# erikszasz/GaussianSplattingRegistration

Hardware: AMD Instinct MI355X
Metric: Gaussians/sec through HEM level + ICP iters/sec, 2x5M-splat pair (higher is better)
Workload: dtype f32 (HEM) / f64 (ICP)

## Files before the change

gaussiansplattingregistration_amd/csrc/hem_select.h:

```cpp
#pragma once
#include "hem_device.h"

namespace gsr {

struct ParentRec;
struct SelectArgs {
    const float4* A;
    const float4* geo;
    const float* Rs;
    const unsigned* plist;
    const unsigned* porder;
    int xcd;
    const int* nheavy;
    int own_lo, own_hi;
    const int* cellStart;
    const float4* Ac;
    const int* cellStartC;
    const int* cellStartI;
    const double* logtab;
    const int* irank;
    const unsigned* ipos;
    int n_irr;
    int ell;
    const GridParams* gp;
// ... 84 lines not shown
    const float kf = 0.5f * (s2 - lf);
    const float margin = 1e-6f * (1.0f + fabsf(lf) + fabsf(s2));
    bool reject = kf > thr;
    const bool need_exact = !(qf >= 4.0f * FLT_MIN && qf <= 0.25f * FLT_MAX) || !(fabsf(s2) <= FLT_MAX) || !(fabsf(kf - thr) > margin);
    if (need_exact) {
        const float k = 0.5f * (s2 - glibc_logf_tab(det_c / det_p, logtab));
        reject = k > thr;
    }
    if (lf_out) *lf_out = lf;
    if (exact_out) *exact_out = need_exact;
    return reject;
}


template <bool IRR>
__device__ __forceinline__ void select_row_span(const SelectArgs& a, const GridParams& g, const f3& pm, const EllClip& ec, bool clip,
                                                float Ra2, int x0, int x1, int ry, int rz, int& s, int& len) {
    const bool edge = ry == 0 || ry == g.gy - 1 || rz == 0 || rz == g.gz - 1;
    const float ylo = ry == 0 ? -FLT_MAX : g.oy + ry * g.c - g.slack, yhi = ry == g.gy - 1 ? FLT_MAX : g.oy + (ry + 1) * g.c + g.slack;
    const float zlo = rz == 0 ? -FLT_MAX : g.oz + rz * g.c - g.slack, zhi = rz == g.gz - 1 ? FLT_MAX : g.oz + (rz + 1) * g.c + g.slack;
    const float dy = fmaxf(0.0f, fmaxf(ylo - pm.y, pm.y - yhi));
    const float dz = fmaxf(0.0f, fmaxf(zlo - pm.z, pm.z - zhi));
    const float rem = Ra2 - dy * dy - dz * dz;
    if (rem >= 0.0f) {
        const float hx = fast_sqrt(rem) * 1.00001f + g.slack;
        float lo = -hx, hi = hx;
        if (clip && !edge) {
            const float cy = 0.5f * (ylo + yhi) - pm.y, cz = 0.5f * (zlo + zhi) - pm.z;
            const float hy = 0.5f * (yhi - ylo), hz = 0.5f * (zhi - zlo);
            const float sc = fast_sqrt(fmaxf(0.0f, ec.k11 * cy * cy + 2.0f * ec.k12 * cy * cz + ec.k22 * cz * cz));
            const float smin = fmaxf(0.0f, sc * 0.999f - ec.kr * fast_sqrt(hy * hy + hz * hz));
// ... 3 lines not shown
            } else {
                const float w = fast_sqrt(rem2 * ec.im00) * 1.001f;
                const float t1 = ec.m01 * cy, t2 = ec.m02 * cz;
                const float xc = -(t1 + t2) * ec.im00;
                const float dl = (fabsf(ec.m01) * hy + fabsf(ec.m02) * hz) * ec.im00 * 1.001f;
                const float pad = g.slack + 1e-5f * fabsf(xc) + 1e-6f * (fabsf(t1) + fabsf(t2)) * ec.im00;
                lo = fmaxf(lo, xc - dl - w - pad);
                hi = fminf(hi, xc + dl + w + pad);
            }
        }
        if (lo <= hi) {
            int xa = cell_of(pm.x + lo, g.ox, g.inv_c, g.gx), xb = cell_of(pm.x + hi, g.ox, g.inv_c, g.gx);
            xa = xa < x0 ? x0 : xa;
            xb = xb > x1 ? x1 : xb;
            const int rowbase = (rz * g.gy + ry) * g.gx;
            int e;
            if (IRR) { s = a.cellStartI[rowbase + xa]; e = a.cellStartI[rowbase + xb + 1]; }
            else { s = a.cellStartC[rowbase + xa]; e = a.cellStartC[rowbase + xb + 1]; }
            len = e - s;
        }
    }
}

__device__ __forceinline__ void make_filter(const s6& Mf, float det_p, float kldThr, int ell, bool parent_regular, ParentRec& pr) {
    EllClip ec;
    ec.on = 0.0f; ec.k11 = ec.k12 = ec.k22 = ec.kr = ec.im00 = ec.m01 = ec.m02 = 0.0f; ec.T = __builtin_inff();
    pr.white = 0.0f;
    pr.u00 = pr.u01 = pr.u02 = pr.u11 = pr.u12 = pr.u22 = 0.0f;
    pr.T1 = __builtin_inff();
    pr.ey = pr.ez = __builtin_inff();
    const double thr2 = 2.0 * (double)kldThr;
    if (parent_regular && thr2 >= 0.0 && thr2 < 1e30) {
        const double m00 = Mf.e00, m01 = Mf.e01, m02 = Mf.e02, m11 = Mf.e11, m12 = Mf.e12, m22 = Mf.e22;
        double detM;
// ... 63 lines not shown
```

gaussiansplattingregistration_amd/csrc/hem_select.hip:

```cpp
#include "hem_select.h"

namespace gsr {

#ifdef GSR_SELECT_PROFILE
__device__ unsigned long long g_sel_prof[1024 * 16];
#endif
struct __attribute__((aligned(16))) ParLds {
    float4 r0;
    float4 r1;
    float4 r2;
    float4 r3;
    float R2;
    int js;
    int64_t base;
};
static_assert(sizeof(ParLds) == 80, "ParLds is read as four float4 and two 8-byte words");

#define SEL_Q3CAP 128
struct Q3 {
    unsigned *j, *rel;
    float *d2, *cd, *op, *det;
    int h, n;
};

__device__ __forceinline__ void select_stage3(const SelectArgs& a, const ParLds* par, int lane, int cnt, Q3& q3) {
    if (lane < cnt) {
        const int k = (q3.h + lane) & (SEL_Q3CAP - 1);
        const unsigned e = q3.j[k];
        const ParLds* pl = par + (e >> SEL_TAG_SHIFT);
        const float distanceDiff = sqrtf(q3.d2[k]);
        const float cdiff = sqrtf(q3.cd[k]);
        const float distWeight = expf(-distanceDiff * distanceDiff / a.tau2);
        const float colorInfluence = expf(-cdiff * cdiff / a.tau2);
        const float L = distWeight * q3.op[k] * colorInfluence * sqrtf(q3.det[k]);
        const int64_t dst = pl->base + (int64_t)q3.rel[k];
        a.pair_child[dst] = e & SEL_TAG_MASK;
        a.pair_wl[dst] = pl->r3.z * ref_clamp(L, FLT_MIN, 1e8f);
    }
    q3.h = (q3.h + cnt) & (SEL_Q3CAP - 1);
    q3.n -= cnt;
}

template <int MODE>
__device__ __forceinline__ void select_stage2(const SelectArgs& a, const ParLds* par, int lane, int cnt, const unsigned* q, int qh,
                                              unsigned& count_v, Q3& q3) {
    SEL_PROF_T(tp2);
    SEL_PROF_CNT(8, 1, lane); SEL_PROF_CNT(9, cnt, lane);
    bool acc = false;
    unsigned e = 0u;
    int k = 0;
    float d2 = 0.0f, cdiff = 0.0f, op = 0.0f, det_c = 0.0f;
    if (lane < cnt) {
        e = q[(qh + lane) & (SEL_QCAP - 1)];
        const int j = (int)(e & SEL_TAG_MASK);
        k = (int)(e >> SEL_TAG_SHIFT);
        const ParLds* pl = par + k;
        const float4 p0 = pl->r0, p1 = pl->r1;
        const float R2 = pl->R2;
        const float4* row = a.geo + 4 * (int64_t)j;
        float4 ca = row[0], cb = row[1], cc = row[2], cd = row[3];
        asm volatile("" : "+v"(ca.x), "+v"(ca.y), "+v"(ca.z), "+v"(ca.w), "+v"(cb.x), "+v"(cb.y), "+v"(cb.z), "+v"(cb.w),
                          "+v"(cc.x), "+v"(cc.y), "+v"(cc.z), "+v"(cc.w), "+v"(cd.x), "+v"(cd.y), "+v"(cd.z), "+v"(cd.w));
        const f3 cm = {ca.x, ca.y, ca.z};
        const f3 ccol = {cc.z, cc.w, cd.x};
        const f3 pm = {p0.x, p0.y, p0.z}, pcol = {p0.w, p1.x, p1.y};
        const f3 d = sub3(cm, pm);
        d2 = dot3(d, d);
        const f3 dc = sub3(ccol, pcol);
        cdiff = dot3(dc, dc);
        if (d2 < R2 && !(cdiff > a.colorThr2)) {
            const float4 p2 = pl->r2, p3 = pl->r3;
            const s6 ccov = {cb.x, cb.y, cb.z, cb.w, cc.x, cc.y};
            const s6 pinv = {p1.z, p1.w, p2.x, p2.y, p2.z, p2.w};
            det_c = cd.w;
            op = cd.y;
            const float smd = dot3(d, mul6(pinv, d));
            const float tr = trace_prod6(pinv, ccov);
            const float s2 = smd + tr - 3.0f;
            if (!kl_gate_rejects(s2, det_c, p3.x, p3.y, a.kldThr, a.logtab)) {
                const bool child_is_parent = (__float_as_uint(ca.w) & 1u) != 0u;
                acc = !(child_is_parent && j != pl->js);
            }
        }
    }
    const unsigned long long m = __ballot(acc);
    const int na = __popcll(m);
    SEL_PROF_CNT(15, na, lane);
    if (na == 0) { SEL_PROF_ADD(2, tp2, lane); return; }
    const int k_lo = __builtin_amdgcn_readfirstlane(k);
    const int k_hi = __builtin_amdgcn_readlane(k, __builtin_amdgcn_readfirstlane(cnt - 1));
    unsigned rel = 0u;
#pragma unroll
    for (int kk = 0; kk < SEL_NP; ++kk) {
        if (kk < k_lo || kk > k_hi) continue;
        const unsigned long long mk = __ballot(acc && k == kk);
        const unsigned ck = (unsigned)__builtin_amdgcn_readlane((int)count_v, kk);
        if (acc && k == kk) rel = ck + (unsigned)mbcnt64(mk, 0);
        if (lane == kk) count_v += (unsigned)__popcll(mk);
    }
    if (MODE == SEL_COUNT) { SEL_PROF_ADD(2, tp2, lane); return; }
    if (acc) {
        const int t = mbcnt64(m, q3.h + q3.n) & (SEL_Q3CAP - 1);
        q3.j[t] = e; q3.rel[t] = rel; q3.d2[t] = d2; q3.cd[t] = cdiff; q3.op[t] = op; q3.det[t] = det_c;
    }
    q3.n += na;
    __builtin_amdgcn_wave_barrier();
    if (q3.n >= 64) select_stage3(a, par, lane, 64, q3);
    __builtin_amdgcn_wave_barrier();
    SEL_PROF_ADD(2, tp2, lane);
}

__global__ __launch_bounds__(256) void k_parent_prep(int P, const unsigned* __restrict__ plist, const float4* __restrict__ geo,
                                                     const float* __restrict__ Rs, float kldThr, int ell, ParentRec* __restrict__ prec) {
    __shared__ ParentRec s_pr[4][64];
    const int lane = threadIdx.x & 63, wv = threadIdx.x >> 6;
    for (int base = blockIdx.x * blockDim.x + (threadIdx.x & ~63); base < P; base += gridDim.x * blockDim.x) {
        const int p = base + lane;
        if (p < P) {
        ParentRec pr;
        pr.js = (int)plist[p];
        const float4* prow = geo + 4 * (int64_t)pr.js;
        const float4 pa = prow[0], pb = prow[1], pc = prow[2], pd = prow[3];
// ... 11 lines not shown
        pr.active = (pr.R2 > 0.0f && pm_finite) ? 1 : 0;
        pr.selfq = (pr.active && (__float_as_uint(pa.w) & 2u)) ? 1 : 0;
        pr.rows = 0;
        s_pr[wv][lane] = pr;
        }
        __builtin_amdgcn_wave_barrier();
        const int nrec = P - base < 64 ? P - base : 64;
        const float4* src = reinterpret_cast<const float4*>(s_pr[wv]);
        float4* dst = reinterpret_cast<float4*>(prec + base);
        for (int t = lane; t < nrec * (int)(sizeof(ParentRec) / 16); t += 64) dst[t] = src[t];
        __builtin_amdgcn_wave_barrier();
    }
}

template <int MODE, bool IRR>
__device__ __forceinline__ void select_scan(const SelectArgs& a, const GridParams& g, const ParentRec& pr, const ParLds* par, unsigned ktag,
                                            const float (&vc)[11], int lane, unsigned long long* bits, unsigned* q, int& qh, int& qn, unsigned& count_v,
                                            Q3& q3, unsigned& cum, unsigned lo, unsigned hi, const int2* rl, int lcnt) {
    const f3 pm = pr.pm;
    const EllClip& ec = pr.ec;
    const bool listed = rl != nullptr;
    bool clip = false;
    int x0 = 0, x1 = 0, y0 = 0, z0 = 0, ny = 1, nrows = lcnt;
    float Ra2 = 0.0f;
    if (!listed) {
        int vz;
        asm volatile("v_mov_b32 %0, 0" : "=v"(vz));
        const auto uni = [vz](int v) { return __builtin_amdgcn_readfirstlane(v + vz); };
        const auto unif = [vz](float v) { return __builtin_bit_cast(float, __builtin_amdgcn_readfirstlane(__builtin_bit_cast(int, v) + vz)); };
        const float Ra = unif(fabsf(pr.R) * 1.00001f + g.slack);
        clip = !IRR && ec.on != 0.0f;
        const float Ry = clip ? fminf(Ra, pr.ey + g.slack) : Ra, Rz = clip ? fminf(Ra, pr.ez + g.slack) : Ra;
        x0 = uni(cell_of(pm.x - Ra, g.ox, g.inv_c, g.gx)); x1 = uni(cell_of(pm.x + Ra, g.ox, g.inv_c, g.gx));
        y0 = uni(cell_of(pm.y - Ry, g.oy, g.inv_c, g.gy));
        const int y1 = uni(cell_of(pm.y + Ry, g.oy, g.inv_c, g.gy));
        z0 = uni(cell_of(pm.z - Rz, g.oz, g.inv_c, g.gz));
        const int z1 = uni(cell_of(pm.z + Rz, g.oz, g.inv_c, g.gz));
        ny = y1 - y0 + 1;
        nrows = ny * (z1 - z0 + 1);
        Ra2 = unif(Ra * Ra);
    }
    const bool white = !IRR && pr.white != 0.0f;
    SEL_PROF_CNT(10, nrows, lane);
    for (int rb = 0; rb < nrows; rb += 64) {
        SEL_PROF_T(tpr);
        SEL_PROF_CNT(11, 1, lane);
        const int r = rb + lane;
        int s = 0, len = 0;
        if (r < nrows) {
            if (listed) { const int2 e = rl[r]; s = e.x; len = e.y; }
            else select_row_span<IRR>(a, g, pm, ec, clip, Ra2, x0, x1, y0 + r % ny, z0 + r / ny, s, len);
        }
        len = len > 0 ? len : 0;
        const unsigned long long nz_m = __ballot(len > 0);
        if (nz_m == 0ull) continue;
        const int incl = wave_incl_scan(len);
        const int pre = incl - len;
        const int total = __builtin_amdgcn_readlane(incl, 63);
        const unsigned cum0 = cum;
        cum += (unsigned)total;
        if (hi <= cum0 || lo >= cum) continue;
        const int b_lo = lo > cum0 ? (int)(lo - cum0) : 0;
        const int b_hi = hi - cum0 < (unsigned)total ? (int)(hi - cum0) : total;
        const int nrb = __popcll(nz_m);
        const int below = mbcnt64(nz_m, 0);
        const int dst = len > 0 ? below : nrb + (lane - below);
// ... 9 lines not shown
            const int seg_end = b_hi < seg0 + SEL_MCAP ? b_hi : seg0 + SEL_MCAP;
            for (int t0 = seg0; t0 < seg_end; t0 += 64 * SEL_U) {
                SEL_PROF_CNT(14, 1, lane);
                SEL_PROF_T(tps);
                float4 ca[SEL_U];
                int jj[SEL_U];
                int left[SEL_U];
#pragma unroll
                for (int u = 0; u < SEL_U; ++u) {
                    const int c0 = t0 + 64 * u;
                    const unsigned long long word = uniform64(bits[(c0 - seg0) >> 6]);
                    const int row = mbcnt64(word >> 1, rows_before - 1 + (int)(word & 1ull));
                    rows_before += __popcll(word);
                    left[u] = seg_end - c0;
                    const int k = c0 + lane + __builtin_amdgcn_ds_bpermute(row << 2, delta);
                    if (IRR) { jj[u] = lane < left[u] ? (int)a.ipos[k] : pr.js; ca[u] = a.A[jj[u]]; }
                    else { jj[u] = k; ca[u] = a.Ac[k]; }
                }
#pragma unroll
                for (int u = 0; u < SEL_U; ++u) {
                    if (left[u] <= 0) continue;
                    const f3 cm = {ca[u].x, ca[u].y, ca[u].z};
                    bool in;
                    if (white) {
                        in = !(white_smd(vc, cm.x, cm.y, cm.z) > vc[9]);
                    } else {
                        const f3 dq = sub3(pm, cm);
                        in = dot3(dq, dq) < pr.R2;
                    }
                    if (!IRR) {
                        in = in && (__float_as_uint(ca[u].w) & 2u);
                        jj[u] = (int)(__float_as_uint(ca[u].w) >> 2);
                    } else {
                        in = in && (!(__float_as_uint(ca[u].w) & 1u) || jj[u] == pr.js);
                    }
                    in = in && lane < left[u];
                    const unsigned long long m = __ballot(in);
                    if (m == 0ull) continue;
                    if (in) q[mbcnt64(m, qh + qn) & (SEL_QCAP - 1)] = (unsigned)jj[u] | ktag;
                    qn += __popcll(m);
                }
                __builtin_amdgcn_wave_barrier();
                SEL_PROF_ADD(4, tps, lane);
                while (qn >= 64) {
                    select_stage2<MODE>(a, par, lane, 64, q, qh, count_v, q3);
                    qh = (qh + 64) & (SEL_QCAP - 1);
                    qn -= 64;
                }
                __builtin_amdgcn_wave_barrier();
            }
            if (mine) bits[rel >> 6] = 0ull;
            __builtin_amdgcn_wave_barrier();
        }
    }
}

__device__ __forceinline__ void select_fill_par(const SelectArgs& a, int p, int64_t base, ParLds* slot) {
    const float4* r = reinterpret_cast<const float4*>(a.prec + p);
    const float4 r0 = r[0], r1 = r[1], r2 = r[2], r3 = r[3];
    slot->r0 = r0; slot->r1 = r1; slot->r2 = r2; slot->r3 = r3;
    slot->R2 = a.prec[p].R2; slot->js = a.prec[p].js; slot->base = base;
}

template <int MODE>
__device__ __forceinline__ void select_parent(const SelectArgs& a, const GridParams& g, int p, int k, unsigned lo, unsigned hi, int lane,
                                              const ParLds* par, unsigned* q, int& qh, int& qn, unsigned long long* bits, unsigned& count_v, Q3& q3) {
    SEL_PROF_T(tp0);
    ParentRec pr;
    {
        typedef unsigned u16v __attribute__((ext_vector_type(16)));
        typedef unsigned u8v __attribute__((ext_vector_type(8)));
        u16v w0, w1; u8v w2;
        const ParentRec* rp = a.prec + p;
        asm volatile("s_load_dwordx16 %0, %3, 0x0\n\ts_load_dwordx16 %1, %3, 0x40\n\ts_load_dwordx8 %2, %3, 0x80\n\ts_waitcnt lgkmcnt(0)"
                     : "=&s"(w0), "=&s"(w1), "=&s"(w2) : "s"(rp) : "memory");
        unsigned raw[40];
        static_assert(sizeof(raw) == sizeof(ParentRec), "the three scalar loads cover the record");
#pragma unroll
        for (int i = 0; i < 16; ++i) { raw[i] = w0[i]; raw[16 + i] = w1[i]; }
#pragma unroll
        for (int i = 0; i < 8; ++i) raw[32 + i] = w2[i];
        __builtin_memcpy(&pr, raw, sizeof(pr));
    }
    float vc[11];
    {
        const float src[11] = {pr.pm.x, pr.pm.y, pr.pm.z, pr.u00, pr.u01, pr.u02, pr.u11, pr.u12, pr.u22, pr.T1, 0.0f};
#pragma unroll
        for (int i = 0; i < 11; ++i) asm volatile("v_mov_b32 %0, %1" : "=v"(vc[i]) : "s"(src[i]));
    }
    const unsigned ktag = (unsigned)k << SEL_TAG_SHIFT;
    unsigned cum = 0;
    if (pr.selfq) {
        cum = 1u;
        if (lo == 0u) {
            if (lane == 0) q[(qh + qn) & (SEL_QCAP - 1)] = (unsigned)pr.js | ktag;
            qn += 1;
        }
        __builtin_amdgcn_wave_barrier();
        if (qn >= 64) {
            select_stage2<MODE>(a, par, lane, 64, q, qh, count_v, q3);
            qh = (qh + 64) & (SEL_QCAP - 1);
            qn -= 64;
        }
    }
    if (pr.active) {
        const int cA = pr.rows & 0xff, cB = (pr.rows >> 8) & 0xff;
        const int2* rlp = (a.rowlist != nullptr && pr.rows < 0) ? a.rowlist + (int64_t)p * (2 * SEL_ROWS) : nullptr;
        select_scan<MODE, false>(a, g, pr, par, ktag, vc, lane, bits, q, qh, qn, count_v, q3, cum, lo, hi,
                                 rlp != nullptr && cA <= SEL_ROWS ? rlp : nullptr, cA);
        if (a.n_irr > 0) select_scan<MODE, true>(a, g, pr, par, ktag, vc, lane, bits, q, qh, qn, count_v, q3, cum, lo, hi,
                                                 rlp != nullptr && cB <= SEL_ROWS ? rlp + SEL_ROWS : nullptr, cB);
    }
    SEL_PROF_ADD(0, tp0, lane);
    SEL_PROF_CNT(7, 1, lane);
}

template <int MODE>
__device__ __forceinline__ void select_flush(const SelectArgs& a, const ParLds* par, int lane, const unsigned* q, int& qh, int& qn,
                                             unsigned& count_v, Q3& q3) {
    while (qn > 0) {
        const int c = qn < 64 ? qn : 64;
        select_stage2<MODE>(a, par, lane, c, q, qh, count_v, q3);
        qh = (qh + c) & (SEL_QCAP - 1);
        qn -= c;
    }
    SEL_PROF_T(tp3);
    if ((MODE == SEL_FILL || MODE == SEL_SPARSE) && q3.n > 0) select_stage3(a, par, lane, q3.n, q3);
    SEL_PROF_ADD(3, tp3, lane);
    __builtin_amdgcn_wave_barrier();
}

template <int MODE, int WPB, bool QUEUE>
__global__ __launch_bounds__(64 * WPB) void k_select(SelectArgs a) {
    __shared__ unsigned s_q[WPB][SEL_QCAP];
    __shared__ unsigned s_q3u[WPB][2][SEL_Q3CAP];
    __shared__ float s_q3f[WPB][4][SEL_Q3CAP];
    __shared__ unsigned long long s_bits[WPB][SEL_MCAP / 64 + SEL_U];
    __shared__ ParLds s_par[WPB][SEL_NP];
    const int lane = threadIdx.x & 63, wv = __builtin_amdgcn_readfirstlane((int)(threadIdx.x >> 6));
    a.logtab = k_logf_tab;
    if (lane < SEL_MCAP / 64 + SEL_U) s_bits[wv][lane] = 0ull;
    unsigned* q = s_q[wv];
    ParLds* par = s_par[wv];
    Q3 q3 = {s_q3u[wv][0], s_q3u[wv][1], s_q3f[wv][0], s_q3f[wv][1], s_q3f[wv][2], s_q3f[wv][3], 0, 0};
    __builtin_amdgcn_wave_barrier();
    const GridParams g = *a.gp;
    int qh = 0, qn = 0;

    if constexpr (QUEUE) {
        const int n_items = a.hq[0];
        const unsigned part = *a.part_p;
        int item = (int)blockIdx.x * WPB + wv;
        while (item < n_items) {
            const uint2 it = a.hitem[item];
            const int p = __builtin_amdgcn_readfirstlane((int)a.porder[it.x]);
            const unsigned lo = (unsigned)__builtin_amdgcn_readfirstlane((int)(it.y * part));
            const unsigned hi = lo + part > lo ? lo + part : 0xffffffffu;
            int64_t base = 0;
            if (MODE == SEL_SPARSE) base = a.poff[p] + lo;
            if (MODE == SEL_SPARSE && a.cap_pairs && (unsigned long long)base + part > a.cap_pairs) {
                if (lane == 0) { a.part_cnt[item] = 0u; *a.abort_p = 1; }
                int nxt0 = 0;
                if (lane == 0) nxt0 = atomicAdd(&a.hq[1], 1);
                item = __builtin_amdgcn_readfirstlane(nxt0);
                continue;
            }
            if (MODE == SEL_FILL) {
                base = a.poff[p];
                for (int k = a.hfirst[p]; k < item; ++k) base += a.part_cnt[k];
            }
            unsigned count_v = 0u;
            if (lane == 0) select_fill_par(a, p, base, par);
            __builtin_amdgcn_wave_barrier();
            select_parent<MODE>(a, g, p, 0, lo, hi, lane, par, q, qh, qn, s_bits[wv], count_v, q3);
            select_flush<MODE>(a, par, lane, q, qh, qn, count_v, q3);
            if (lane == 0 && (MODE == SEL_COUNT || MODE == SEL_SPARSE)) {
                a.part_cnt[item] = count_v;
                atomicAdd(&a.pcnt[p], count_v);
            }
            int nxt = 0;
            if (lane == 0) nxt = atomicAdd(&a.hq[1], 1);
            item = __builtin_amdgcn_readfirstlane(nxt);
            __builtin_amdgcn_wave_barrier();
        }
    } else {
        SEL_PROF_T(tpk);
        const int np = a.np;
        const int ppb = WPB * np;
        const int nheavy = a.nheavy ? *a.nheavy : 0;
        const int nblk = (a.P + ppb - 1) / ppb;
        const int hb = ((nheavy + ppb - 1) / ppb + 7) & ~7;
        const int bid = block_slot((int)blockIdx.x, nblk, hb < nblk ? hb : nblk, a.xcd);
        if (bid < 0) return;
        const int slot0 = (bid * WPB + wv) * np;
        int p_v = -1;
        if (lane < np) {
// ... 9 lines not shown
                    } else {
                        p_v = p;
                        select_fill_par(a, p, base, par + lane);
                    }
                }
            }
        }
        unsigned long long todo = __ballot(p_v >= 0);
        unsigned count_v = 0u;
        __builtin_amdgcn_wave_barrier();
        SEL_PROF_ADD(5, tpk, lane);
        while (todo != 0ull) {
            const int k = __builtin_ctzll(todo);
            todo &= todo - 1ull;
            const int p = __builtin_amdgcn_readlane(p_v, k);
            select_parent<MODE>(a, g, p, k, 0u, 0xffffffffu, lane, par, q, qh, qn, s_bits[wv], count_v, q3);
        }
        SEL_PROF_T(tpf);
        select_flush<MODE>(a, par, lane, q, qh, qn, count_v, q3);
        SEL_PROF_ADD(6, tpf, lane);
        if (p_v >= 0 && (MODE == SEL_COUNT || MODE == SEL_SPARSE)) a.pcnt[p_v] = count_v;
    }
}

__global__ __launch_bounds__(256) void k_spans(SelectArgs a) {
    const int sub = threadIdx.x & 15;
    const int p = (int)(((int64_t)blockIdx.x * blockDim.x + threadIdx.x) >> 4);
    if (p >= a.P) return;
    unsigned long long scanned = 0;
    int selfq = 0;
    int nA = 0, nB = 0;
    if (p >= a.own_lo && p < a.own_hi) {
        const GridParams g = *a.gp;
        const float4* rq = reinterpret_cast<const float4*>(a.prec + p);
        float4 q0 = rq[0], q3 = rq[3], q6 = rq[6], q7 = rq[7], q8 = rq[8], q9 = rq[9];
        asm volatile("" : "+v"(q0.x), "+v"(q0.y), "+v"(q0.z), "+v"(q3.w), "+v"(q6.y), "+v"(q6.z), "+v"(q6.w), "+v"(q7.x), "+v"(q7.y), "+v"(q7.z), "+v"(q7.w),
// ... 14 lines not shown
            }
            n += __popc(gm);
        };
        if (rp->active) {
            const float Ra = fabsf(rp->R) * 1.00001f + g.slack;
            const float Ra2 = Ra * Ra;
            const int x0 = cell_of(pm.x - Ra, g.ox, g.inv_c, g.gx), x1 = cell_of(pm.x + Ra, g.ox, g.inv_c, g.gx);
            {
                const bool clip = ec.on != 0.0f;
                const float Ry = clip ? fminf(Ra, rp->ey + g.slack) : Ra, Rz = clip ? fminf(Ra, rp->ez + g.slack) : Ra;
                const int y0 = cell_of(pm.y - Ry, g.oy, g.inv_c, g.gy), y1 = cell_of(pm.y + Ry, g.oy, g.inv_c, g.gy);
                const int z0 = cell_of(pm.z - Rz, g.oz, g.inv_c, g.gz), z1 = cell_of(pm.z + Rz, g.oz, g.inv_c, g.gz);
                const int ny = y1 - y0 + 1, nrows = ny * (z1 - z0 + 1);
                for (int r = sub; r < nrows; r += 16) {
                    int s = 0, len = 0;
                    select_row_span<false>(a, g, pm, ec, clip, Ra2, x0, x1, y0 + r % ny, z0 + r / ny, s, len);
                    scanned += (unsigned long long)(len > 0 ? len : 0);
                    keep_span(0, s, len, nA);
                }
            }
            if (a.n_irr > 0) {
                const int y0 = cell_of(pm.y - Ra, g.oy, g.inv_c, g.gy), y1 = cell_of(pm.y + Ra, g.oy, g.inv_c, g.gy);
                const int z0 = cell_of(pm.z - Ra, g.oz, g.inv_c, g.gz), z1 = cell_of(pm.z + Ra, g.oz, g.inv_c, g.gz);
                const int ny = y1 - y0 + 1, nrows = ny * (z1 - z0 + 1);
                for (int r = sub; r < nrows; r += 16) {
                    int s = 0, len = 0;
                    select_row_span<true>(a, g, pm, ec, false, Ra2, x0, x1, y0 + r % ny, z0 + r / ny, s, len);
                    scanned += (unsigned long long)(len > 0 ? len : 0);
                    keep_span(1, s, len, nB);
                }
            }
        }
    }
    for (int o = 8; o > 0; o >>= 1) scanned += __shfl_xor(scanned, o);
    if (selfq) scanned += 1ull;
    if (sub == 0) {
        a.pcap[p] = (unsigned)(scanned > 0xffffffffull ? 0xffffffffull : scanned);
        if (a.rowlist) const_cast<ParentRec*>(a.prec)[p].rows = (int)(0x80000000u | (unsigned)(nA > SEL_ROWS ? 0xff : nA) | ((unsigned)(nB > SEL_ROWS ? 0xff : nB) << 8));
    }
}

void launch_parent_prep(hipStream_t st, int P, const unsigned* plist, const float4* geo, const float* Rs, float kldThr, int ell, ParentRec* prec) {
// ... 40 lines not shown
```

gaussiansplattingregistration_amd/csrc/icp.hip:

```cpp
#include "gsr_common.h"
#include "gsr_normals.h"
#include "gsr_solve.h"
#include "gsr_features.h"
#include "gsr_oneshot.h"

#include <float.h>
#include <math.h>
#include <stdlib.h>
#include <string.h>
#include <chrono>
#include <vector>

#include <rocprim/rocprim.hpp>

namespace gsr {
#ifndef GSR_ICP_MERGE_BS
#define GSR_ICP_MERGE_BS 1024
#define GSR_ICP_MERGE_IPT 4
#endif
using icp_merge_cfg = rocprim::merge_sort_config<512, GSR_ICP_MERGE_BS, GSR_ICP_MERGE_IPT, 128, 128, 4>;
using icp_sort_cfg = rocprim::radix_sort_config<rocprim::default_config, icp_merge_cfg,
                                                rocprim::radix_sort_onesweep_config<rocprim::kernel_config<1024, 16>, rocprim::kernel_config<1024, 16>, 11,
                                                                                    rocprim::block_radix_rank_algorithm::match>>;

// ... 194 lines not shown
    const double d = ((v < lo && k > 0) ? lo - v : ((v > hi && k < g - 1) ? v - hi : 0.0)) * 0.999999999 - eps;
    return d > 0.0 ? d : 0.0;
}

__device__ __forceinline__ void icp_consider(const float4 q, int j, double px, double py, double pz, double& bd, int& best, unsigned& best_i) {
    const double dx = px - (double)q.x, dy = py - (double)q.y, dz = pz - (double)q.z;
    const double d2 = dx * dx + dy * dy + dz * dz;
    const unsigned qi = __float_as_uint(q.w);
    if (d2 < bd || (d2 == bd && qi < best_i)) { bd = d2; best = j; best_i = qi; }
}

#define ICP_BLOCK_CROWDED 24
#ifndef ICP_ROW_BATCH
#define ICP_ROW_BATCH 4
#endif
template <int BLOCK>
__device__ __forceinline__ int icp_nearest(const IcpGrid& g, const int* __restrict__ cellStart,
                                           const float4* __restrict__ Tq, double px, double py, double pz, double& best_d2,
                                           double bound2 = 1.0 / 0.0) {
    int best = -1;
    unsigned best_i = 0xffffffffu;
    double bd = bound2;
    if (!(px == px) || !(py == py) || !(pz == pz)) { best_d2 = 1.0 / 0.0; return -1; }
    {
        const double ex = fmax(fmax(g.bx0 - px, px - g.bx1), 0.0), ey = fmax(fmax(g.by0 - py, py - g.by1), 0.0), ez = fmax(fmax(g.bz0 - pz, pz - g.bz1), 0.0);
        if ((ex * ex + ey * ey + ez * ez) * 0.999999999 >= bound2) { best_d2 = bound2; return -1; }
    }
    const int cx = icp_cell(px, g.ox, g.inv_c, g.gx), cy = icp_cell(py, g.oy, g.inv_c, g.gy), cz = icp_cell(pz, g.oz, g.inv_c, g.gz);
    const double eps = 1e-13 * (fabs(px) + fabs(py) + fabs(pz) + fabs(g.ox) + fabs(g.oy) + fabs(g.oz) + g.c * (double)(g.gx + g.gy + g.gz));
    int r0 = 0;
    if (BLOCK == 1 && g.rings >= 1) {
        int rs[9], re[9];
        const int xa = cx - 1 > 0 ? cx - 1 : 0, xb = cx + 1 < g.gx - 1 ? cx + 1 : g.gx - 1;
#pragma unroll
        for (int t = 0; t < 9; ++t) {
            const int z = cz + t / 3 - 1, y = cy + t % 3 - 1;
            const bool ok = z >= 0 && z < g.gz && y >= 0 && y < g.gy;
            const int rowbase = ok ? (z * g.gy + y) * g.gx : 0;
            rs[t] = ok ? cellStart[rowbase + xa] : 0;
            re[t] = ok ? cellStart[rowbase + xb + 1] : 0;
// ... 709 lines not shown


struct IcpState {
    double T[16];
    double fit, rmse;
    double ctr[3], nsg, rel_fit, rel_rmse;
    int iters, done, max_iter, kind, evals;
};

__device__ __forceinline__ bool icp_state_done(const IcpState* st) { return st->done != 0; }
__device__ __forceinline__ void icp_state_T(const IcpState* st, double T[12]) {
#pragma unroll
    for (int i = 0; i < 12; ++i) T[i] = st->T[i];
}

template <int KIND, int BLOCK, int FUSE>
__global__ __launch_bounds__(256, (FUSE != 0 && KIND != 2) ? 3 : 1) void k_icp_accumulate_dev(int64_t ns, const float* __restrict__ src, IcpState* st,
                                                            IcpGrid g, const int* __restrict__ cellStart, const int* __restrict__ nn_j,
                                                            const float4* __restrict__ Tq, const double* __restrict__ Tn,
                                                            const double* __restrict__ Sc, ColorArgs ca, double max_corr2,
                                                            int loss, double kparam, double* partials, unsigned* ticket,
                                                            double* acc_out, int nb_logical) {
    constexpr int fuse = FUSE;
    constexpr bool PERSIST = FUSE == 3;
    constexpr int NACC = KIND == 0 ? 17 : 30;
    __shared__ int s_last;
    __shared__ int s_stop;
    __shared__ double s_x[8][GSR_ICP_ACC_LEN];
    __shared__ IcpState s_st;
    const IcpRange rg = icp_block_range(ns, nb_logical < 0 ? -nb_logical : nb_logical, FUSE == 0 && nb_logical > 0);
    for (unsigned ev = 0;; ++ev) {
    double T[12];
    if constexpr (PERSIST) {
        if (threadIdx.x == 0) s_stop = __hip_atomic_load(&st->done, __ATOMIC_RELAXED, __HIP_MEMORY_SCOPE_AGENT) | (int)__hip_atomic_load(ticket + 2, __ATOMIC_RELAXED, __HIP_MEMORY_SCOPE_AGENT);
        __syncthreads();
        if (s_stop) return;
#pragma unroll
        for (int i = 0; i < 12; ++i) T[i] = __hip_atomic_load(&st->T[i], __ATOMIC_RELAXED, __HIP_MEMORY_SCOPE_AGENT);
    } else {
    if (st->done) {
        if (fuse == 2 && blockIdx.x == 0 && threadIdx.x < GSR_ICP_ACC_LEN) acc_out[threadIdx.x] = 0.0;
        return;
    }
#pragma unroll
    for (int i = 0; i < 12; ++i) T[i] = st->T[i];
    }
    double acc[NACC];
#pragma unroll
    for (int k = 0; k < NACC; ++k) acc[k] = 0.0;
    if (rg.row < 0) return;
    for (int64_t i = rg.lo + threadIdx.x; i < rg.hi; i += blockDim.x) {
        const double x = (double)src[3 * i], y = (double)src[3 * i + 1], z = (double)src[3 * i + 2];
        const double px = T[0] * x + T[1] * y + T[2] * z + T[3];
        const double py = T[4] * x + T[5] * y + T[6] * z + T[7];
        const double pz = T[8] * x + T[9] * y + T[10] * z + T[11];
        int j;
        if (nn_j) {
            j = nn_j[i];
            if (j < 0) continue;
        } else {
            double dd;
            j = icp_nearest<BLOCK>(g, cellStart, Tq, px, py, pz, dd, max_corr2);
            if (j < 0 || !(dd < max_corr2)) continue;
        }
        const float4 q = Tq[j];
        const double qx = (double)q.x, qy = (double)q.y, qz = (double)q.z;
        const double ddx = px - qx, ddy = py - qy, ddz = pz - qz;
        const double d2 = ddx * ddx + ddy * ddy + ddz * ddz;
        acc[0] += 1.0;
        acc[1] += d2;
        if constexpr (KIND == 0) {
            const double ax = px - g.cx, ay = py - g.cy, az = pz - g.cz;
            const double bx = qx - g.cx, by = qy - g.cy, bz = qz - g.cz;
            acc[2] += ax; acc[3] += ay; acc[4] += az;
            acc[5] += bx; acc[6] += by; acc[7] += bz;
            acc[8] += ax * bx; acc[9] += ax * by; acc[10] += ax * bz;
            acc[11] += ay * bx; acc[12] += ay * by; acc[13] += ay * bz;
            acc[14] += az * bx; acc[15] += az * by; acc[16] += az * bz;
        } else if constexpr (KIND == 2) {
            icp_gicp_rows<NACC>(acc, T, px, py, pz, qx, qy, qz, Sc + 6 * i, Tn + 6 * (int64_t)j, loss, kparam);
        } else if constexpr (KIND == 3) {
            icp_colored_rows<NACC>(acc, ca, px, py, pz, qx, qy, qz, Tn[3 * (int64_t)j], Tn[3 * (int64_t)j + 1], Tn[3 * (int64_t)j + 2], i, j, loss, kparam);
        } else {
            const double nx = Tn[3 * (int64_t)j], ny = Tn[3 * (int64_t)j + 1], nz = Tn[3 * (int64_t)j + 2];
            const double r = (px - qx) * nx + (py - qy) * ny + (pz - qz) * nz;
            const double w = icp_weight(loss, kparam, r);
            const double J[6] = {py * nz - pz * ny, pz * nx - px * nz, px * ny - py * nx, nx, ny, nz};
            int t = 2;
#pragma unroll
            for (int a = 0; a < 6; ++a)
#pragma unroll
                for (int b = a; b < 6; ++b) acc[t++] += J[a] * w * J[b];
#pragma unroll
            for (int a = 0; a < 6; ++a) acc[23 + a] += J[a] * w * r;
            acc[29] += r * r;
        }
    }
    block_reduce_store<NACC, FUSE != 0>(acc, partials, rg.row);
    if constexpr (FUSE == 0) return;
    if (threadIdx.x < 64) {
        asm volatile("s_waitcnt vmcnt(0)" ::: "memory");
        if (threadIdx.x == 0) {
            __builtin_amdgcn_fence(__ATOMIC_RELEASE, "agent");
            const unsigned t = __hip_atomic_fetch_add(ticket, 1u, __ATOMIC_ACQ_REL, __HIP_MEMORY_SCOPE_AGENT);
            s_last = t == (PERSIST ? (ev + 1u) * gridDim.x - 1u : gridDim.x - 1u) ? 1 : 0;
            if (s_last) __builtin_amdgcn_fence(__ATOMIC_ACQUIRE, "agent");
        }
    }
    __syncthreads();
    if (s_last) {
        if constexpr (PERSIST) {
            if (threadIdx.x < sizeof(IcpState) / 4)
// ... 1002 lines not shown
```

Before: 569.2 million.

## Re-read kernel arguments from kernarg segment to cut register pressure

Stops passing the SelectArgs struct and grid parameters through the HEM selection helpers. Kernel-argument fields and the grid are now re-fetched on demand from the kernarg segment with scalar loads. In the non-fused ICP accumulate kernel, the transform, bounding box, normals pointer and loss parameters are likewise reloaded inside the loop instead of being held live across it. The aim is to lower SGPR/VGPR pressure and spills, at the cost of extra scalar loads per iteration, and it relies on hard-coded kernarg offsets matching the ABI layout.

```diff
diff --git a/gaussiansplattingregistration_amd/csrc/hem_select.h b/gaussiansplattingregistration_amd/csrc/hem_select.h
--- a/gaussiansplattingregistration_amd/csrc/hem_select.h
+++ b/gaussiansplattingregistration_amd/csrc/hem_select.h
@@ -122,7 +122,7 @@
 
 
 template <bool IRR>
-__device__ __forceinline__ void select_row_span(const SelectArgs& a, const GridParams& g, const f3& pm, const EllClip& ec, bool clip,
+__device__ __forceinline__ void select_row_span(const int* __restrict__ cst, const GridParams& g, const f3& pm, const EllClip& ec, bool clip,
                                                 float Ra2, int x0, int x1, int ry, int rz, int& s, int& len) {
     const bool edge = ry == 0 || ry == g.gy - 1 || rz == 0 || rz == g.gz - 1;
     const float ylo = ry == 0 ? -FLT_MAX : g.oy + ry * g.c - g.slack, yhi = ry == g.gy - 1 ? FLT_MAX : g.oy + (ry + 1) * g.c + g.slack;
@@ -156,10 +156,8 @@
             xa = xa < x0 ? x0 : xa;
             xb = xb > x1 ? x1 : xb;
             const int rowbase = (rz * g.gy + ry) * g.gx;
-            int e;
-            if (IRR) { s = a.cellStartI[rowbase + xa]; e = a.cellStartI[rowbase + xb + 1]; }
-            else { s = a.cellStartC[rowbase + xa]; e = a.cellStartC[rowbase + xb + 1]; }
-            len = e - s;
+            s = cst[rowbase + xa];
+            len = cst[rowbase + xb + 1] - s;
         }
     }
 }
diff --git a/gaussiansplattingregistration_amd/csrc/hem_select.hip b/gaussiansplattingregistration_amd/csrc/hem_select.hip
--- a/gaussiansplattingregistration_amd/csrc/hem_select.hip
+++ b/gaussiansplattingregistration_amd/csrc/hem_select.hip
@@ -5,6 +5,28 @@
 #ifdef GSR_SELECT_PROFILE
 __device__ unsigned long long g_sel_prof[1024 * 16];
 #endif
+typedef const __attribute__((address_space(4))) SelectArgs* SelKargs;
+__device__ __forceinline__ SelKargs select_kargs() {
+    SelKargs ka = (SelKargs)__builtin_amdgcn_kernarg_segment_ptr();
+    asm volatile("" : "+s"(ka));
+    return ka;
+}
+
+__device__ __forceinline__ GridParams select_grid(const GridParams* gp) {
+    typedef unsigned u8v __attribute__((ext_vector_type(8)));
+    typedef unsigned u2v __attribute__((ext_vector_type(2)));
+    static_assert(sizeof(GridParams) == 40, "GridParams is fetched as 8 + 2 dwords");
+    u8v w0; u2v w1;
+    asm volatile("s_load_dwordx8 %0, %2, 0x0\n\ts_load_dwordx2 %1, %2, 0x20\n\ts_waitcnt lgkmcnt(0)" : "=&s"(w0), "=&s"(w1) : "s"(gp) : "memory");
+    unsigned raw[10];
+#pragma unroll
+    for (int i = 0; i < 8; ++i) raw[i] = w0[i];
+    raw[8] = w1[0]; raw[9] = w1[1];
+    GridParams g;
+    __builtin_memcpy(&g, raw, sizeof(g));
+    return g;
+}
+
 struct __attribute__((aligned(16))) ParLds {
     float4 r0;
     float4 r1;
@@ -23,26 +45,30 @@
     int h, n;
 };
 
-__device__ __forceinline__ void select_stage3(const SelectArgs& a, const ParLds* par, int lane, int cnt, Q3& q3) {
+__device__ __forceinline__ void select_stage3(const ParLds* par, int lane, int cnt, Q3& q3) {
     if (lane < cnt) {
+        const SelKargs ka = select_kargs();
+        const float tau2 = ka->tau2;
+        unsigned* const pair_child = ka->pair_child;
+        float* const pair_wl = ka->pair_wl;
         const int k = (q3.h + lane) & (SEL_Q3CAP - 1);
         const unsigned e = q3.j[k];
         const ParLds* pl = par + (e >> SEL_TAG_SHIFT);
         const float distanceDiff = sqrtf(q3.d2[k]);
         const float cdiff = sqrtf(q3.cd[k]);
-        const float distWeight = expf(-distanceDiff * distanceDiff / a.tau2);
-        const float colorInfluence = expf(-cdiff * cdiff / a.tau2);
+        const float distWeight = expf(-distanceDiff * distanceDiff / tau2);
+        const float colorInfluence = expf(-cdiff * cdiff / tau2);
         const float L = distWeight * q3.op[k] * colorInfluence * sqrtf(q3.det[k]);
         const int64_t dst = pl->base + (int64_t)q3.rel[k];
-        a.pair_child[dst] = e & SEL_TAG_MASK;
-        a.pair_wl[dst] = pl->r3.z * ref_clamp(L, FLT_MIN, 1e8f);
+        pair_child[dst] = e & SEL_TAG_MASK;
+        pair_wl[dst] = pl->r3.z * ref_clamp(L, FLT_MIN, 1e8f);
     }
     q3.h = (q3.h + cnt) & (SEL_Q3CAP - 1);
     q3.n -= cnt;
 }
 
 template <int MODE>
-__device__ __forceinline__ void select_stage2(const SelectArgs& a, const ParLds* par, int lane, int cnt, const unsigned* q, int qh,
+__device__ __forceinline__ void select_stage2(const ParLds* par, int lane, int cnt, const unsigned* q, int qh,
                                               unsigned& count_v, Q3& q3) {
     SEL_PROF_T(tp2);
     SEL_PROF_CNT(8, 1, lane); SEL_PROF_CNT(9, cnt, lane);
@@ -57,7 +83,9 @@
         const ParLds* pl = par + k;
         const float4 p0 = pl->r0, p1 = pl->r1;
         const float R2 = pl->R2;
-        const float4* row = a.geo + 4 * (int64_t)j;
+        const SelKargs ka = select_kargs();
+        const float colorThr2 = ka->colorThr2, kldThr = ka->kldThr;
+        const float4* row = ka->geo + 4 * (int64_t)j;
         float4 ca = row[0], cb = row[1], cc = row[2], cd = row[3];
         asm volatile("" : "+v"(ca.x), "+v"(ca.y), "+v"(ca.z), "+v"(ca.w), "+v"(cb.x), "+v"(cb.y), "+v"(cb.z), "+v"(cb.w),
                           "+v"(cc.x), "+v"(cc.y), "+v"(cc.z), "+v"(cc.w), "+v"(cd.x), "+v"(cd.y), "+v"(cd.z), "+v"(cd.w));
@@ -68,7 +96,7 @@
         d2 = dot3(d, d);
         const f3 dc = sub3(ccol, pcol);
         cdiff = dot3(dc, dc);
-        if (d2 < R2 && !(cdiff > a.colorThr2)) {
+        if (d2 < R2 && !(cdiff > colorThr2)) {
             const float4 p2 = pl->r2, p3 = pl->r3;
             const s6 ccov = {cb.x, cb.y, cb.z, cb.w, cc.x, cc.y};
             const s6 pinv = {p1.z, p1.w, p2.x, p2.y, p2.z, p2.w};
@@ -77,7 +105,7 @@
             const float smd = dot3(d, mul6(pinv, d));
             const float tr = trace_prod6(pinv, ccov);
             const float s2 = smd + tr - 3.0f;
-            if (!kl_gate_rejects(s2, det_c, p3.x, p3.y, a.kldThr, a.logtab)) {
+            if (!kl_gate_rejects(s2, det_c, p3.x, p3.y, kldThr, k_logf_tab)) {
                 const bool child_is_parent = (__float_as_uint(ca.w) & 1u) != 0u;
                 acc = !(child_is_parent && j != pl->js);
             }
@@ -105,7 +133,7 @@
     }
     q3.n += na;
     __builtin_amdgcn_wave_barrier();
-    if (q3.n >= 64) select_stage3(a, par, lane, 64, q3);
+    if (q3.n >= 64) select_stage3(par, lane, 64, q3);
     __builtin_amdgcn_wave_barrier();
     SEL_PROF_ADD(2, tp2, lane);
 }
@@ -147,16 +175,20 @@
 }
 
 template <int MODE, bool IRR>
-__device__ __forceinline__ void select_scan(const SelectArgs& a, const GridParams& g, const ParentRec& pr, const ParLds* par, unsigned ktag,
+__device__ __forceinline__ void select_scan(const ParentRec& pr, const ParLds* par, unsigned ktag,
                                             const float (&vc)[11], int lane, unsigned long long* bits, unsigned* q, int& qh, int& qn, unsigned& count_v,
                                             Q3& q3, unsigned& cum, unsigned lo, unsigned hi, const int2* rl, int lcnt) {
-    const f3 pm = pr.pm;
+    const f3 pm = {vc[0], vc[1], vc[2]};
     const EllClip& ec = pr.ec;
     const bool listed = rl != nullptr;
     bool clip = false;
     int x0 = 0, x1 = 0, y0 = 0, z0 = 0, ny = 1, nrows = lcnt;
     float Ra2 = 0.0f;
+    const SelKargs ka = select_kargs();
+    const float4* const Ac = IRR ? ka->A : ka->Ac;
+    const unsigned* const ipos = IRR ? ka->ipos : nullptr;
     if (!listed) {
+        const GridParams g = select_grid(ka->gp);
         int vz;
         asm volatile("v_mov_b32 %0, 0" : "=v"(vz));
         const auto uni = [vz](int v) { return __builtin_amdgcn_readfirstlane(v + vz); };
@@ -180,9 +212,16 @@
         SEL_PROF_CNT(11, 1, lane);
         const int r = rb + lane;
         int s = 0, len = 0;
+        GridParams g = {};
+        const int* cst = nullptr;
+        if (!listed) {
+            const SelKargs kr = select_kargs();
+            g = select_grid(kr->gp);
+            cst = IRR ? kr->cellStartI : kr->cellStartC;
+        }
         if (r < nrows) {
             if (listed) { const int2 e = rl[r]; s = e.x; len = e.y; }
-            else select_row_span<IRR>(a, g, pm, ec, clip, Ra2, x0, x1, y0 + r % ny, z0 + r / ny, s, len);
+            else select_row_span<IRR>(cst, g, pm, ec, clip, Ra2, x0, x1, y0 + r % ny, z0 + r / ny, s, len);
         }
         len = len > 0 ? len : 0;
         const unsigned long long nz_m = __ballot(len > 0);
@@ -222,8 +261,8 @@
                     rows_before += __popcll(word);
                     left[u] = seg_end - c0;
                     const int k = c0 + lane + __builtin_amdgcn_ds_bpermute(row << 2, delta);
-                    if (IRR) { jj[u] = lane < left[u] ? (int)a.ipos[k] : pr.js; ca[u] = a.A[jj[u]]; }
-                    else { jj[u] = k; ca[u] = a.Ac[k]; }
+                    if (IRR) { jj[u] = lane < left[u] ? (int)ipos[k] : pr.js; ca[u] = Ac[jj[u]]; }
+                    else { jj[u] = k; ca[u] = Ac[k]; }
                 }
 #pragma unroll
                 for (int u = 0; u < SEL_U; ++u) {
@@ -251,7 +290,7 @@
                 __builtin_amdgcn_wave_barrier();
                 SEL_PROF_ADD(4, tps, lane);
                 while (qn >= 64) {
-                    select_stage2<MODE>(a, par, lane, 64, q, qh, count_v, q3);
+                    select_stage2<MODE>(par, lane, 64, q, qh, count_v, q3);
                     qh = (qh + 64) & (SEL_QCAP - 1);
                     qn -= 64;
                 }
@@ -271,7 +310,7 @@
 }
 
 template <int MODE>
-__device__ __forceinline__ void select_parent(const SelectArgs& a, const GridParams& g, int p, int k, unsigned lo, unsigned hi, int lane,
+__device__ __forceinline__ void select_parent(int p, int k, unsigned lo, unsigned hi, int lane,
                                               const ParLds* par, unsigned* q, int& qh, int& qn, unsigned long long* bits, unsigned& count_v, Q3& q3) {
     SEL_PROF_T(tp0);
     ParentRec pr;
@@ -279,7 +318,7 @@
         typedef unsigned u16v __attribute__((ext_vector_type(16)));
         typedef unsigned u8v __attribute__((ext_vector_type(8)));
         u16v w0, w1; u8v w2;
-        const ParentRec* rp = a.prec + p;
+        const ParentRec* rp = select_kargs()->prec + p;
         asm volatile("s_load_dwordx16 %0, %3, 0x0\n\ts_load_dwordx16 %1, %3, 0x40\n\ts_load_dwordx8 %2, %3, 0x80\n\ts_waitcnt lgkmcnt(0)"
                      : "=&s"(w0), "=&s"(w1), "=&s"(w2) : "s"(rp) : "memory");
         unsigned raw[40];
@@ -306,17 +345,18 @@
         }
         __builtin_amdgcn_wave_barrier();
         if (qn >= 64) {
-            select_stage2<MODE>(a, par, lane, 64, q, qh, count_v, q3);
+            select_stage2<MODE>(par, lane, 64, q, qh, count_v, q3);
             qh = (qh + 64) & (SEL_QCAP - 1);
             qn -= 64;
         }
     }
     if (pr.active) {
         const int cA = pr.rows & 0xff, cB = (pr.rows >> 8) & 0xff;
-        const int2* rlp = (a.rowlist != nullptr && pr.rows < 0) ? a.rowlist + (int64_t)p * (2 * SEL_ROWS) : nullptr;
-        select_scan<MODE, false>(a, g, pr, par, ktag, vc, lane, bits, q, qh, qn, count_v, q3, cum, lo, hi,
+        const int2* const rowlist = select_kargs()->rowlist;
+        const int2* rlp = (rowlist != nullptr && pr.rows < 0) ? rowlist + (int64_t)p * (2 * SEL_ROWS) : nullptr;
+        select_scan<MODE, false>(pr, par, ktag, vc, lane, bits, q, qh, qn, count_v, q3, cum, lo, hi,
                                  rlp != nullptr && cA <= SEL_ROWS ? rlp : nullptr, cA);
-        if (a.n_irr > 0) select_scan<MODE, true>(a, g, pr, par, ktag, vc, lane, bits, q, qh, qn, count_v, q3, cum, lo, hi,
+        if (select_kargs()->n_irr > 0) select_scan<MODE, true>(pr, par, ktag, vc, lane, bits, q, qh, qn, count_v, q3, cum, lo, hi,
                                                  rlp != nullptr && cB <= SEL_ROWS ? rlp + SEL_ROWS : nullptr, cB);
     }
     SEL_PROF_ADD(0, tp0, lane);
@@ -324,16 +364,16 @@
 }
 
 template <int MODE>
-__device__ __forceinline__ void select_flush(const SelectArgs& a, const ParLds* par, int lane, const unsigned* q, int& qh, int& qn,
+__device__ __forceinline__ void select_flush(const ParLds* par, int lane, const unsigned* q, int& qh, int& qn,
                                              unsigned& count_v, Q3& q3) {
     while (qn > 0) {
         const int c = qn < 64 ? qn : 64;
-        select_stage2<MODE>(a, par, lane, c, q, qh, count_v, q3);
+        select_stage2<MODE>(par, lane, c, q, qh, count_v, q3);
         qh = (qh + c) & (SEL_QCAP - 1);
         qn -= c;
     }
     SEL_PROF_T(tp3);
-    if ((MODE == SEL_FILL || MODE == SEL_SPARSE) && q3.n > 0) select_stage3(a, par, lane, q3.n, q3);
+    if ((MODE == SEL_FILL || MODE == SEL_SPARSE) && q3.n > 0) select_stage3(par, lane, q3.n, q3);
     SEL_PROF_ADD(3, tp3, lane);
     __builtin_amdgcn_wave_barrier();
 }
@@ -346,48 +386,47 @@
     __shared__ unsigned long long s_bits[WPB][SEL_MCAP / 64 + SEL_U];
     __shared__ ParLds s_par[WPB][SEL_NP];
     const int lane = threadIdx.x & 63, wv = __builtin_amdgcn_readfirstlane((int)(threadIdx.x >> 6));
-    a.logtab = k_logf_tab;
     if (lane < SEL_MCAP / 64 + SEL_U) s_bits[wv][lane] = 0ull;
     unsigned* q = s_q[wv];
     ParLds* par = s_par[wv];
     Q3 q3 = {s_q3u[wv][0], s_q3u[wv][1], s_q3f[wv][0], s_q3f[wv][1], s_q3f[wv][2], s_q3f[wv][3], 0, 0};
     __builtin_amdgcn_wave_barrier();
-    const GridParams g = *a.gp;
     int qh = 0, qn = 0;
 
     if constexpr (QUEUE) {
-        const int n_items = a.hq[0];
-        const unsigned part = *a.part_p;
         int item = (int)blockIdx.x * WPB + wv;
-        while (item < n_items) {
-            const uint2 it = a.hitem[item];
-            const int p = __builtin_amdgcn_readfirstlane((int)a.porder[it.x]);
+        while (item < select_kargs()->hq[0]) {
+            const SelKargs ka = select_kargs();
+            const unsigned part = *ka->part_p;
+            const uint2 it = ka->hitem[item];
+            const int p = __builtin_amdgcn_readfirstlane((int)ka->porder[it.x]);
             const unsigned lo = (unsigned)__builtin_amdgcn_readfirstlane((int)(it.y * part));
             const unsigned hi = lo + part > lo ? lo + part : 0xffffffffu;
             int64_t base = 0;
-            if (MODE == SEL_SPARSE) base = a.poff[p] + lo;
-            if (MODE == SEL_SPARSE && a.cap_pairs && (unsigned long long)base + part > a.cap_pairs) {
-                if (lane == 0) { a.part_cnt[item] = 0u; *a.abort_p = 1; }
+            if (MODE == SEL_SPARSE) base = ka->poff[p] + lo;
+            if (MODE == SEL_SPARSE && ka->cap_pairs && (unsigned long long)base + part > ka->cap_pairs) {
+                if (lane == 0) { ka->part_cnt[item] = 0u; *ka->abort_p = 1; }
                 int nxt0 = 0;
-                if (lane == 0) nxt0 = atomicAdd(&a.hq[1], 1);
+                if (lane == 0) nxt0 = atomicAdd(&ka->hq[1], 1);
                 item = __builtin_amdgcn_readfirstlane(nxt0);
                 continue;
             }
             if (MODE == SEL_FILL) {
-                base = a.poff[p];
-                for (int k = a.hfirst[p]; k < item; ++k) base += a.part_cnt[k];
+                base = ka->poff[p];
+                for (int k = ka->hfirst[p]; k < item; ++k) base += ka->part_cnt[k];
             }
             unsigned count_v = 0u;
             if (lane == 0) select_fill_par(a, p, base, par);
             __builtin_amdgcn_wave_barrier();
-            select_parent<MODE>(a, g, p, 0, lo, hi, lane, par, q, qh, qn, s_bits[wv], count_v, q3);
-            select_flush<MODE>(a, par, lane, q, qh, qn, count_v, q3);
+            select_parent<MODE>(p, 0, lo, hi, lane, par, q, qh, qn, s_bits[wv], count_v, q3);
+            select_flush<MODE>(par, lane, q, qh, qn, count_v, q3);
+            const SelKargs kb = select_kargs();
             if (lane == 0 && (MODE == SEL_COUNT || MODE == SEL_SPARSE)) {
-                a.part_cnt[item] = count_v;
-                atomicAdd(&a.pcnt[p], count_v);
+                kb->part_cnt[item] = count_v;
+                atomicAdd(&kb->pcnt[p], count_v);
             }
             int nxt = 0;
-            if (lane == 0) nxt = atomicAdd(&a.hq[1], 1);
+            if (lane == 0) nxt = atomicAdd(&kb->hq[1], 1);
             item = __builtin_amdgcn_readfirstlane(nxt);
             __builtin_amdgcn_wave_barrier();
         }
@@ -427,12 +466,12 @@
             const int k = __builtin_ctzll(todo);
             todo &= todo - 1ull;
             const int p = __builtin_amdgcn_readlane(p_v, k);
-            select_parent<MODE>(a, g, p, k, 0u, 0xffffffffu, lane, par, q, qh, qn, s_bits[wv], count_v, q3);
+            select_parent<MODE>(p, k, 0u, 0xffffffffu, lane, par, q, qh, qn, s_bits[wv], count_v, q3);
         }
         SEL_PROF_T(tpf);
-        select_flush<MODE>(a, par, lane, q, qh, qn, count_v, q3);
+        select_flush<MODE>(par, lane, q, qh, qn, count_v, q3);
         SEL_PROF_ADD(6, tpf, lane);
-        if (p_v >= 0 && (MODE == SEL_COUNT || MODE == SEL_SPARSE)) a.pcnt[p_v] = count_v;
+        if (p_v >= 0 && (MODE == SEL_COUNT || MODE == SEL_SPARSE)) select_kargs()->pcnt[p_v] = count_v;
     }
 }
 
@@ -477,7 +516,7 @@
                 const int ny = y1 - y0 + 1, nrows = ny * (z1 - z0 + 1);
                 for (int r = sub; r < nrows; r += 16) {
                     int s = 0, len = 0;
-                    select_row_span<false>(a, g, pm, ec, clip, Ra2, x0, x1, y0 + r % ny, z0 + r / ny, s, len);
+                    select_row_span<false>(a.cellStartC, g, pm, ec, clip, Ra2, x0, x1, y0 + r % ny, z0 + r / ny, s, len);
                     scanned += (unsigned long long)(len > 0 ? len : 0);
                     keep_span(0, s, len, nA);
                 }
@@ -488,7 +527,7 @@
                 const int ny = y1 - y0 + 1, nrows = ny * (z1 - z0 + 1);
                 for (int r = sub; r < nrows; r += 16) {
                     int s = 0, len = 0;
-                    select_row_span<true>(a, g, pm, ec, false, Ra2, x0, x1, y0 + r % ny, z0 + r / ny, s, len);
+                    select_row_span<true>(a.cellStartI, g, pm, ec, false, Ra2, x0, x1, y0 + r % ny, z0 + r / ny, s, len);
                     scanned += (unsigned long long)(len > 0 ? len : 0);
                     keep_span(1, s, len, nB);
                 }
diff --git a/gaussiansplattingregistration_amd/csrc/icp.hip b/gaussiansplattingregistration_amd/csrc/icp.hip
--- a/gaussiansplattingregistration_amd/csrc/icp.hip
+++ b/gaussiansplattingregistration_amd/csrc/icp.hip
@@ -232,16 +232,19 @@
 #ifndef ICP_ROW_BATCH
 #define ICP_ROW_BATCH 4
 #endif
-template <int BLOCK>
+typedef const __attribute__((address_space(4))) IcpGrid* IcpGridK;
+template <int BLOCK, bool KBOX = false>
 __device__ __forceinline__ int icp_nearest(const IcpGrid& g, const int* __restrict__ cellStart,
                                            const float4* __restrict__ Tq, double px, double py, double pz, double& best_d2,
-                                           double bound2 = 1.0 / 0.0) {
+                                           double bound2 = 1.0 / 0.0, IcpGridK gk = nullptr) {
     int best = -1;
     unsigned best_i = 0xffffffffu;
     double bd = bound2;
     if (!(px == px) || !(py == py) || !(pz == pz)) { best_d2 = 1.0 / 0.0; return -1; }
     {
-        const double ex = fmax(fmax(g.bx0 - px, px - g.bx1), 0.0), ey = fmax(fmax(g.by0 - py, py - g.by1), 0.0), ez = fmax(fmax(g.bz0 - pz, pz - g.bz1), 0.0);
+        const double bx0 = KBOX ? gk->bx0 : g.bx0, by0 = KBOX ? gk->by0 : g.by0, bz0 = KBOX ? gk->bz0 : g.bz0;
+        const double bx1 = KBOX ? gk->bx1 : g.bx1, by1 = KBOX ? gk->by1 : g.by1, bz1 = KBOX ? gk->bz1 : g.bz1;
+        const double ex = fmax(fmax(bx0 - px, px - bx1), 0.0), ey = fmax(fmax(by0 - py, py - by1), 0.0), ez = fmax(fmax(bz0 - pz, pz - bz1), 0.0);
         if ((ex * ex + ey * ey + ez * ez) * 0.999999999 >= bound2) { best_d2 = bound2; return -1; }
     }
     const int cx = icp_cell(px, g.ox, g.inv_c, g.gx), cy = icp_cell(py, g.oy, g.inv_c, g.gy), cz = icp_cell(pz, g.oz, g.inv_c, g.gz);
@@ -981,6 +984,18 @@
     for (int i = 0; i < 12; ++i) T[i] = st->T[i];
 }
 
+struct IcpAccArgs {
+    int64_t ns; const float* src; IcpState* st; IcpGrid g; const int* cellStart; const int* nn_j; const float4* Tq; const double* Tn;
+    const double* Sc; ColorArgs ca; double max_corr2; int loss; double kparam; double* partials; unsigned* ticket; double* acc_out; int nb_logical;
+};
+static_assert(offsetof(IcpAccArgs, g) == 24 && offsetof(IcpAccArgs, Tn) == 184 && offsetof(IcpAccArgs, loss) == 248 && offsetof(IcpAccArgs, kparam) == 256 &&
+              offsetof(IcpAccArgs, partials) == 264 && offsetof(IcpAccArgs, nb_logical) == 288, "the offsets in the kernel's .amdhsa metadata (.offset of every argument)");
+typedef const __attribute__((address_space(4))) IcpAccArgs* IcpAccKargs;
+__device__ __forceinline__ IcpAccKargs icp_acc_kargs() {
+    IcpAccKargs ka = (IcpAccKargs)__builtin_amdgcn_kernarg_segment_ptr();
+    asm volatile("" : "+s"(ka));
+    return ka;
+}
 template <int KIND, int BLOCK, int FUSE>
 __global__ __launch_bounds__(256, (FUSE != 0 && KIND != 2) ? 3 : 1) void k_icp_accumulate_dev(int64_t ns, const float* __restrict__ src, IcpState* st,
                                                             IcpGrid g, const int* __restrict__ cellStart, const int* __restrict__ nn_j,
@@ -990,6 +1005,7 @@
                                                             double* acc_out, int nb_logical) {
     constexpr int fuse = FUSE;
     constexpr bool PERSIST = FUSE == 3;
+    constexpr bool LATE = FUSE == 0 && KIND != 2;
     constexpr int NACC = KIND == 0 ? 17 : 30;
     __shared__ int s_last;
     __shared__ int s_stop;
@@ -1009,8 +1025,10 @@
         if (fuse == 2 && blockIdx.x == 0 && threadIdx.x < GSR_ICP_ACC_LEN) acc_out[threadIdx.x] = 0.0;
         return;
     }
-#pragma unroll
-    for (int i = 0; i < 12; ++i) T[i] = st->T[i];
+    if constexpr (!LATE) {
+#pragma unroll
+        for (int i = 0; i < 12; ++i) T[i] = st->T[i];
+    }
     }
     double acc[NACC];
 #pragma unroll
@@ -1018,6 +1036,11 @@
     if (rg.row < 0) return;
     for (int64_t i = rg.lo + threadIdx.x; i < rg.hi; i += blockDim.x) {
         const double x = (double)src[3 * i], y = (double)src[3 * i + 1], z = (double)src[3 * i + 2];
+        if constexpr (LATE) {
+            const IcpState* stl = icp_acc_kargs()->st;
+#pragma unroll
+            for (int k = 0; k < 12; ++k) T[k] = stl->T[k];
+        }
         const double px = T[0] * x + T[1] * y + T[2] * z + T[3];
         const double py = T[4] * x + T[5] * y + T[6] * z + T[7];
         const double pz = T[8] * x + T[9] * y + T[10] * z + T[11];
@@ -1027,8 +1050,16 @@
             if (j < 0) continue;
         } else {
             double dd;
-            j = icp_nearest<BLOCK>(g, cellStart, Tq, px, py, pz, dd, max_corr2);
+            if constexpr (LATE) j = icp_nearest<BLOCK, true>(g, cellStart, Tq, px, py, pz, dd, max_corr2, &icp_acc_kargs()->g);
+            else j = icp_nearest<BLOCK>(g, cellStart, Tq, px, py, pz, dd, max_corr2);
             if (j < 0 || !(dd < max_corr2)) continue;
+        }
+        const double* Tn_u = Tn;
+        int loss_u = loss;
+        double kparam_u = kparam;
+        if constexpr (LATE) {
+            const IcpAccKargs kb = icp_acc_kargs();
+            Tn_u = kb->Tn; loss_u = kb->loss; kparam_u = kb->kparam;
         }
         const float4 q = Tq[j];
         const double qx = (double)q.x, qy = (double)q.y, qz = (double)q.z;
@@ -1045,13 +1076,13 @@
             acc[11] += ay * bx; acc[12] += ay * by; acc[13] += ay * bz;
             acc[14] += az * bx; acc[15] += az * by; acc[16] += az * bz;
         } else if constexpr (KIND == 2) {
-            icp_gicp_rows<NACC>(acc, T, px, py, pz, qx, qy, qz, Sc + 6 * i, Tn + 6 * (int64_t)j, loss, kparam);
+            icp_gicp_rows<NACC>(acc, T, px, py, pz, qx, qy, qz, Sc + 6 * i, Tn_u + 6 * (int64_t)j, loss_u, kparam_u);
         } else if constexpr (KIND == 3) {
-            icp_colored_rows<NACC>(acc, ca, px, py, pz, qx, qy, qz, Tn[3 * (int64_t)j], Tn[3 * (int64_t)j + 1], Tn[3 * (int64_t)j + 2], i, j, loss, kparam);
+            icp_colored_rows<NACC>(acc, ca, px, py, pz, qx, qy, qz, Tn_u[3 * (int64_t)j], Tn_u[3 * (int64_t)j + 1], Tn_u[3 * (int64_t)j + 2], i, j, loss_u, kparam_u);
         } else {
-            const double nx = Tn[3 * (int64_t)j], ny = Tn[3 * (int64_t)j + 1], nz = Tn[3 * (int64_t)j + 2];
+            const double nx = Tn_u[3 * (int64_t)j], ny = Tn_u[3 * (int64_t)j + 1], nz = Tn_u[3 * (int64_t)j + 2];
             const double r = (px - qx) * nx + (py - qy) * ny + (pz - qz) * nz;
-            const double w = icp_weight(loss, kparam, r);
+            const double w = icp_weight(loss_u, kparam_u, r);
             const double J[6] = {py * nz - pz * ny, pz * nx - px * nz, px * ny - py * nx, nx, ny, nz};
             int t = 2;
 #pragma unroll
@@ -1063,6 +1094,7 @@
             acc[29] += r * r;
         }
     }
+    if constexpr (LATE) { block_reduce_store<NACC, false>(acc, icp_acc_kargs()->partials, rg.row); return; }
     block_reduce_store<NACC, FUSE != 0>(acc, partials, rg.row);
     if constexpr (FUSE == 0) return;
     if (threadIdx.x < 64) {
```

Result: no change. 569.9 million, median of 3 (+0.1%).
